# YuriPaglierani/Movie-Recommender-System-with-GNNs

Hardware: AMD Instinct MI355X
Metric: edges propagated/sec (K=3, d=64) (higher is better)
Workload: dtype fp32

## Files before the change

### include/lgcn.h

```cpp
#ifndef LGCN_H
#define LGCN_H

#include <stddef.h>
#include <stdint.h>

#ifdef __cplusplus
extern "C" {
#endif

typedef void* lgcn_stream_t;

#define LGCN_ABI_VERSION 11

#define LGCN_OK 0
#define LGCN_E_ARG (-1)
#define LGCN_E_WORKSPACE (-2)
#define LGCN_E_UNSUPPORTED (-3)

typedef struct {
    int64_t beg;
    int32_t len;
    int32_t dst;
} lgcn_item_t;

// ... 63 lines not shown
              float* partial, int32_t mode, float div, float mul,
              lgcn_stream_t stream);

int lgcn_spmm_items(const lgcn_item_t* items, int64_t n_items,
                    const lgcn_split_t* splits, int64_t n_splits,
                    const int32_t* col, const float* val, int64_t N, int32_t d,
                    const float* x_lo, const float* x_hi, int64_t x_split,
                    const float* e_lo, const float* e_hi, int64_t e_split,
                    float* y,
                    float* acc_lo, float* acc_hi, int64_t acc_split,
                    float* partial, int32_t mode, float div, float mul,
                    lgcn_stream_t stream);
int lgcn_spmm_combine(const lgcn_item_t* items, int64_t n_items,
                      const lgcn_split_t* splits, int64_t n_splits,
                      const int32_t* col, const float* val, int64_t N, int32_t d,
                      const float* x_lo, const float* x_hi, int64_t x_split,
                      const float* e_lo, const float* e_hi, int64_t e_split,
                      float* y,
                      float* acc_lo, float* acc_hi, int64_t acc_split,
                      float* partial, int32_t mode, float div, float mul,
                      lgcn_stream_t stream);
int lgcn_coalesce_workspace_size(int64_t P, int64_t N, size_t* bytes);
int lgcn_coalesce_undirected(const int64_t* src, const int64_t* dst, int64_t P, int64_t N, int64_t* out_row,
                             int64_t* out_col, int64_t* out_count, int64_t* err_count, void* ws, size_t ws_bytes,
                             lgcn_stream_t stream);

int lgcn_slice_schedule_workspace_size(int64_t E, int64_t N, int32_t S, int32_t chunk, size_t* bytes,
                                       int64_t* items_cap);
int lgcn_slice_schedule_build(const int64_t* rowptr, const int32_t* col, int64_t N, int64_t E,
                              const int64_t* bounds, int32_t S, int32_t chunk, const uint8_t* row_mask,
                              lgcn_item_t* items, int64_t items_cap,
                              int64_t* offsets, lgcn_split_t* splits, int64_t splits_cap, int64_t* counts,
                              void* ws, size_t ws_bytes, lgcn_stream_t stream);

int lgcn_spmm_run(const lgcn_item_t* items, int64_t n_items, const lgcn_split_t* splits, int64_t n_splits,
                  const int32_t* col, const float* val, int64_t N, int32_t d, const float* x_lo, const float* x_hi,
                  int64_t x_split, const float* e_lo, const float* e_hi, int64_t e_split, float* y, float* acc_lo,
                  float* acc_hi, int64_t acc_split, float* partial, int32_t mode, float div, float mul,
                  lgcn_stream_t stream, float* run);

int lgcn_spmm_run_slices(const lgcn_item_t* items, const int64_t* slice_offsets, int32_t S, const int32_t* col,
                         const float* val, int64_t N, int32_t d, const float* x_lo, const float* x_hi,
                         int64_t x_split, const float* e_lo, const float* e_hi, int64_t e_split, float* y,
                         float* acc_lo, float* acc_hi, int64_t acc_split, float* partial, int32_t mode, float div,
                         float mul, lgcn_stream_t stream, float* run);

int lgcn_spmm_blocksplit(const lgcn_item_t* items, int64_t n_items, const lgcn_split_t* splits, int64_t n_splits,
                         const int32_t* col, const float* val, int64_t N, int32_t d, const float* x_lo,
                         const float* x_hi, int64_t x_split, const float* e_lo, const float* e_hi, int64_t e_split,
                         float* y, float* acc_lo, float* acc_hi, int64_t acc_split, float* partial, int32_t mode,
                         float div, float mul, lgcn_stream_t stream, const lgcn_item_t* chunks);

typedef struct {
    const lgcn_item_t* items;
    int64_t n_items;
    const lgcn_split_t* splits;
    int64_t n_splits;
    const int32_t* col;
    const float* val;
    const float* x_lo;
    const float* x_hi;
    int64_t x_split;
    const float* e_lo;
    const float* e_hi;
    int64_t e_split;
    float* y;
// ... 279 lines not shown
```

### movie-recommender-system-with-gnns_amd/csrc/lgcn_plan.hip

```cpp

#include <hipcub/hipcub.hpp>

#include "lgcn_common.h"

using namespace lgcn;

namespace {

__global__ void k_prep_keys(const int64_t* __restrict__ key, const int64_t* __restrict__ other,
                            int64_t E, int64_t N, int32_t* __restrict__ key32,
                            int32_t* __restrict__ eid, unsigned long long* __restrict__ err) {
    const int64_t stride = int64_t(gridDim.x) * blockDim.x;
    unsigned long long bad_local = 0;
    for (int64_t e = int64_t(blockIdx.x) * blockDim.x + threadIdx.x; e < E; e += stride) {
        const int64_t k = key[e];
        const int64_t o = other[e];
        const bool bad = (k < 0) | (k >= N) | (o < 0) | (o >= N);
        bad_local += bad;
        key32[e] = bad ? 0 : static_cast<int32_t>(k);
        eid[e] = static_cast<int32_t>(e);
    }
    if (bad_local) atomicAdd(err, bad_local);
}

// ... 239 lines not shown
                sp.row = static_cast<int32_t>(i);
                sp.pbeg = part_off[i];
                sp.pcnt = n_part[i];
                sp.pad = 0;
                splits[split_off[i]] = sp;
            }
        }
        if (i == N - 1) {
            counts[0] = item_off[i] + n_items[i];
            counts[1] = split_off[i] + n_split[i];
            counts[2] = part_off[i] + n_part[i];
        }
    }
}

__global__ void k_slice_offsets(const uint32_t* __restrict__ skeys, int64_t n, int S, int64_t* __restrict__ offsets) {
    const int s = blockIdx.x * blockDim.x + threadIdx.x;
    if (s > S) return;
    const uint32_t key = static_cast<uint32_t>(s) << 24;
    int64_t lo = 0, hi = n;
    while (lo < hi) {
        const int64_t mid = (lo + hi) >> 1;
        if (skeys[mid] < key) lo = mid + 1;
        else hi = mid;
    }
    offsets[s] = lo;
}

int64_t slice_items_cap(int64_t E, int64_t N, int S, int32_t chunk) {
    const int64_t segs = E < N * int64_t(S) ? E : N * int64_t(S);
    return segs + E / chunk + N + 1;
}

__global__ void k_pair_keys(const int64_t* __restrict__ src, const int64_t* __restrict__ dst, int64_t P, int64_t N,
                            unsigned long long* __restrict__ keys, int32_t* __restrict__ bad) {
    const int64_t stride = int64_t(gridDim.x) * blockDim.x;
    for (int64_t i = int64_t(blockIdx.x) * blockDim.x + threadIdx.x; i < P; i += stride) {
        const int64_t a = src[i], b = dst[i];
        if (a < 0 || a >= N || b < 0 || b >= N) atomicOr(bad, 1);
        const int64_t ca = a < 0 ? 0 : (a >= N ? N - 1 : a);
        const int64_t cb = b < 0 ? 0 : (b >= N ? N - 1 : b);
        keys[i] = static_cast<unsigned long long>(ca) * static_cast<unsigned long long>(N) + static_cast<unsigned long long>(cb);
        keys[P + i] = static_cast<unsigned long long>(cb) * static_cast<unsigned long long>(N) + static_cast<unsigned long long>(ca);
    }
}

__global__ void k_unique_flags(const unsigned long long* __restrict__ k, int64_t n, int32_t* __restrict__ flag) {
    const int64_t stride = int64_t(gridDim.x) * blockDim.x;
    for (int64_t i = int64_t(blockIdx.x) * blockDim.x + threadIdx.x; i < n; i += stride)
        flag[i] = (i == 0 || k[i] != k[i - 1]) ? 1 : 0;
}

__global__ void k_unique_scatter(const unsigned long long* __restrict__ k, const int32_t* __restrict__ flag,
                                 const int32_t* __restrict__ pos, int64_t n, int64_t N, int64_t* __restrict__ row,
                                 int64_t* __restrict__ col, int64_t* __restrict__ count) {
    const int64_t stride = int64_t(gridDim.x) * blockDim.x;
    for (int64_t i = int64_t(blockIdx.x) * blockDim.x + threadIdx.x; i < n; i += stride) {
        if (flag[i]) {
            const unsigned long long v = k[i];
            row[pos[i]] = static_cast<int64_t>(v / static_cast<unsigned long long>(N));
            col[pos[i]] = static_cast<int64_t>(v % static_cast<unsigned long long>(N));
        }
        if (i == n - 1) count[0] = pos[i] + flag[i];
    }
}

// ... 368 lines not shown
    int32_t* i_in = c.take<int32_t>(cap);
    int32_t* i_out = c.take<int32_t>(cap);
    size_t cub_bytes = sched_cub_bytes(E, N, chunk);
    void* cub_tmp = c.take<char>(cub_bytes);
    if (!c.ok) return fail(LGCN_E_WORKSPACE, "lgcn_schedule_build: workspace %zu < %zu", ws_bytes, c.used);

    const unsigned g = grid_for(N, kBlock, 8192);
    k_sched_count<<<g, kBlock, 0, s>>>(rowptr, N, chunk, row_mask, n_items, n_part, n_split);
    if (int rc = check_launch("k_sched_count")) return rc;
    size_t t = cub_bytes;
    if (int rc = check_hip(hipcub::DeviceScan::ExclusiveSum(cub_tmp, t, n_items, item_off, static_cast<int>(N), s), "scan items")) return rc;
    t = cub_bytes;
    if (int rc = check_hip(hipcub::DeviceScan::ExclusiveSum(cub_tmp, t, n_part, part_off, static_cast<int>(N), s), "scan parts")) return rc;
    t = cub_bytes;
    if (int rc = check_hip(hipcub::DeviceScan::ExclusiveSum(cub_tmp, t, n_split, split_off, static_cast<int>(N), s), "scan splits")) return rc;
    const uint32_t pad_key = 0xFFFFFFFFu;
    k_fill_u32<<<grid_for(cap, kBlock, 8192), kBlock, 0, s>>>(k_in, cap, pad_key);
    if (int rc = check_launch("k_fill_u32")) return rc;
    k_fill_u32<<<grid_for(cap, kBlock, 8192), kBlock, 0, s>>>(reinterpret_cast<uint32_t*>(i_in), cap, 0u);
    if (int rc = check_launch("k_fill_u32")) return rc;
    k_sched_fill<<<g, kBlock, 0, s>>>(rowptr, N, chunk, side_split, n_items, item_off, n_part, part_off, n_split,
                                      split_off, raw, k_in, i_in, splits, counts);
    if (int rc = check_launch("k_sched_fill")) return rc;
    t = cub_bytes;
    if (int rc = check_hip(hipcub::DeviceRadixSort::SortPairs(cub_tmp, t, k_in, k_out, i_in, i_out,
                                                              static_cast<int>(cap), 0, 32, s),
                           "SortPairs(schedule)"))
        return rc;
    k_sched_gather<<<grid_for(cap, kBlock, 8192), kBlock, 0, s>>>(raw, i_out, cap, items);
    return check_launch("k_sched_gather");
}


int lgcn_slice_schedule_workspace_size(int64_t E, int64_t N, int32_t S, int32_t chunk, size_t* bytes,
                                       int64_t* items_cap) {
    if (!bytes || E < 0 || N < 0 || S < 1 || S > 250 || chunk < 1)
        return fail(LGCN_E_ARG, "lgcn_slice_schedule_workspace_size: bad args");
    const int64_t cap = slice_items_cap(E, N, S, chunk);
    if (items_cap) *items_cap = cap;
    size_t a = 0, b = 0, c = 0;
    (void)hipcub::DeviceScan::ExclusiveSum(nullptr, a, (const int64_t*)nullptr, (int64_t*)nullptr,
                                           static_cast<int>(N > 0 ? N : 1));
    (void)hipcub::DeviceScan::ExclusiveSum(nullptr, b, (const int32_t*)nullptr, (int32_t*)nullptr,
                                           static_cast<int>(N > 0 ? N : 1));
    (void)hipcub::DeviceRadixSort::SortPairs(nullptr, c, (const uint32_t*)nullptr, (uint32_t*)nullptr,
                                             (const int32_t*)nullptr, (int32_t*)nullptr, static_cast<int>(cap), 0,
                                             32);
    size_t m = a > b ? a : b;
    m = m > c ? m : c;
    Carver cv{nullptr, 0};
    cv.take<int64_t>(N);
    cv.take<int64_t>(N);
    cv.take<int32_t>(N);
    cv.take<int32_t>(N);
    cv.take<int32_t>(N);
    cv.take<int32_t>(N);
    cv.take<lgcn_item_t>(cap);
    cv.take<uint32_t>(cap);
    cv.take<uint32_t>(cap);
    cv.take<int32_t>(cap);
    cv.take<int32_t>(cap);
    cv.take<char>(m);
    *bytes = cv.used + 256;
    return LGCN_OK;
}

int lgcn_slice_schedule_build(const int64_t* rowptr, const int32_t* col, int64_t N, int64_t E,
                              const int64_t* bounds, int32_t S, int32_t chunk, const uint8_t* row_mask,
                              lgcn_item_t* items, int64_t items_cap,
                              int64_t* offsets, lgcn_split_t* splits, int64_t splits_cap, int64_t* counts,
                              void* ws, size_t ws_bytes, lgcn_stream_t stream) {
    if (!rowptr || !bounds || !counts || !offsets || N <= 0 || E < 0 || S < 1 || S > 250 || chunk < 1 ||
        chunk >= (1 << 24) || (E > 0 && !col))
        return fail(LGCN_E_ARG, "lgcn_slice_schedule_build: bad args");
    if (N > INT32_MAX || E > INT32_MAX) return fail(LGCN_E_UNSUPPORTED, "slice schedule: sizes exceed int32");
    hipStream_t s = as_stream(stream);
    const int64_t cap = slice_items_cap(E, N, S, chunk);
    if (!items || items_cap < cap || !splits || splits_cap < N)
        return fail(LGCN_E_ARG, "lgcn_slice_schedule_build: items_cap %lld < %lld or splits_cap %lld < %lld",
                    (long long)items_cap, (long long)cap, (long long)splits_cap, (long long)N);
    Carver c{static_cast<char*>(ws), ws_bytes};
    int64_t* n_items = c.take<int64_t>(N);
    int64_t* item_off = c.take<int64_t>(N);
    int32_t* n_part = c.take<int32_t>(N);
    int32_t* part_off = c.take<int32_t>(N);
    int32_t* n_split = c.take<int32_t>(N);
    int32_t* split_off = c.take<int32_t>(N);
    lgcn_item_t* raw = c.take<lgcn_item_t>(cap);
    uint32_t* k_in = c.take<uint32_t>(cap);
    uint32_t* k_out = c.take<uint32_t>(cap);
    int32_t* i_in = c.take<int32_t>(cap);
    int32_t* i_out = c.take<int32_t>(cap);
    size_t a = 0, b = 0, cb = 0;
    (void)hipcub::DeviceScan::ExclusiveSum(nullptr, a, (const int64_t*)nullptr, (int64_t*)nullptr, static_cast<int>(N));
    (void)hipcub::DeviceScan::ExclusiveSum(nullptr, b, (const int32_t*)nullptr, (int32_t*)nullptr, static_cast<int>(N));
    (void)hipcub::DeviceRadixSort::SortPairs(nullptr, cb, (const uint32_t*)nullptr, (uint32_t*)nullptr,
                                             (const int32_t*)nullptr, (int32_t*)nullptr, static_cast<int>(cap), 0, 32);
    size_t cub_bytes = a > b ? a : b;
    cub_bytes = cub_bytes > cb ? cub_bytes : cb;
    void* cub_tmp = c.take<char>(cub_bytes);
    if (!c.ok) return fail(LGCN_E_WORKSPACE, "lgcn_slice_schedule_build: workspace %zu < %zu", ws_bytes, c.used);
    if (int rc = check_hip(hipMemsetAsync(counts, 0, 4 * sizeof(int64_t), s), "memset counts")) return rc;
    const unsigned g = grid_for(N, kBlock, 8192);
    k_slice_count<<<grid_for(N * 64, kBlock, 8192), kBlock, 0, s>>>(rowptr, col, N, bounds, S, chunk, row_mask,
                                                                     n_items, n_part,
                                                                     n_split,
                                       reinterpret_cast<int32_t*>(counts + 3));
    if (int rc = check_launch("k_slice_count")) return rc;
    size_t t = cub_bytes;
    if (int rc = check_hip(hipcub::DeviceScan::ExclusiveSum(cub_tmp, t, n_items, item_off, static_cast<int>(N), s), "scan items")) return rc;
    t = cub_bytes;
    if (int rc = check_hip(hipcub::DeviceScan::ExclusiveSum(cub_tmp, t, n_part, part_off, static_cast<int>(N), s), "scan parts")) return rc;
    t = cub_bytes;
    if (int rc = check_hip(hipcub::DeviceScan::ExclusiveSum(cub_tmp, t, n_split, split_off, static_cast<int>(N), s), "scan splits")) return rc;
    k_fill_u32<<<grid_for(cap, kBlock, 8192), kBlock, 0, s>>>(k_in, cap, 0xFFFFFFFFu);
    if (int rc = check_launch("k_fill_u32")) return rc;
    k_fill_u32<<<grid_for(cap, kBlock, 8192), kBlock, 0, s>>>(reinterpret_cast<uint32_t*>(i_in), cap, 0u);
    if (int rc = check_launch("k_fill_u32")) return rc;
    k_slice_fill<<<g, kBlock, 0, s>>>(rowptr, col, N, bounds, S, chunk, row_mask, n_items, item_off, n_part, part_off, n_split,
                                      split_off, raw, k_in, i_in, splits, counts);
    if (int rc = check_launch("k_slice_fill")) return rc;
    t = cub_bytes;
    if (int rc = check_hip(hipcub::DeviceRadixSort::SortPairs(cub_tmp, t, k_in, k_out, i_in, i_out,
                                                              static_cast<int>(cap), 0, 32, s),
                           "SortPairs(slice schedule)"))
        return rc;
    k_sched_gather<<<grid_for(cap, kBlock, 8192), kBlock, 0, s>>>(raw, i_out, cap, items);
    if (int rc = check_launch("k_sched_gather")) return rc;
    k_slice_offsets<<<1, 256, 0, s>>>(k_out, cap, S, offsets);
    return check_launch("k_slice_offsets");
}


int lgcn_coalesce_workspace_size(int64_t P, int64_t N, size_t* bytes) {
    if (!bytes || P < 0 || N < 0) return fail(LGCN_E_ARG, "lgcn_coalesce_workspace_size: bad args");
    if (2 * P > INT32_MAX || N > (int64_t(1) << 31)) return fail(LGCN_E_UNSUPPORTED, "coalesce: sizes exceed int32");
    const int64_t n = 2 * P > 0 ? 2 * P : 1;
    Carver c{nullptr, 0};
    c.take<unsigned long long>(n);
    c.take<unsigned long long>(n);
    c.take<int32_t>(n);
    c.take<int32_t>(n);
    c.take<int32_t>(1);
    c.take<char>(coalesce_cub_bytes(n, coalesce_bits(N > 1 ? N : 2)));
    *bytes = c.used + 256;
    return LGCN_OK;
}

int lgcn_coalesce_undirected(const int64_t* src, const int64_t* dst, int64_t P, int64_t N, int64_t* out_row,
                             int64_t* out_col, int64_t* out_count, int64_t* err_count, void* ws, size_t ws_bytes,
                             lgcn_stream_t stream) {
    if (P < 0 || N <= 0 || !out_count || !err_count || (P > 0 && (!src || !dst || !out_row || !out_col)))
        return fail(LGCN_E_ARG, "lgcn_coalesce_undirected: bad args");
    if (2 * P > INT32_MAX) return fail(LGCN_E_UNSUPPORTED, "coalesce: sizes exceed int32");
    hipStream_t s = as_stream(stream);
    if (int rc = check_hip(hipMemsetAsync(out_count, 0, sizeof(int64_t), s), "memset count")) return rc;
    if (int rc = check_hip(hipMemsetAsync(err_count, 0, sizeof(int64_t), s), "memset err")) return rc;
    if (P == 0) return LGCN_OK;
    const int64_t n = 2 * P;
    const int bits = coalesce_bits(N > 1 ? N : 2);
    Carver c{static_cast<char*>(ws), ws_bytes};
    auto* k_in = c.take<unsigned long long>(n);
    auto* k_out = c.take<unsigned long long>(n);
// ... 25 lines not shown
```

### movie-recommender-system-with-gnns_amd/lgcn_amd/_ffi.py

```python
from __future__ import annotations

import ctypes
import os
import pathlib

_HERE = pathlib.Path(__file__).resolve().parent
LIB_PATH = _HERE / "liblgcn.so"

EPI_INIT = 0
EPI_ADD = 1
EPI_FINAL_ACC = 2
EPI_FINAL_E = 3
EPI_STORE = 4
EPI_SCALE = 5

E_ARG, E_WORKSPACE, E_UNSUPPORTED = -1, -2, -3

ITEM_BYTES = 16
SPLIT_BYTES = 16
ABI_VERSION = 11
DIGEST_BLOCKS = 1024
RANKED_MAX_K = 1024
RANKED_MAX_CAP = 262144
RANKED_REPEATS = -1
# ... 112 lines not shown
    "lgcn_rows_accumulate": ([_vp, _vp, _i64, _i64, _i64, _vp, _vp, _vp, _i64, _i32, _f32, _vp], ctypes.c_int),
    "lgcn_recall_width": ([_i32, _vp, _vp], ctypes.c_int),
    "lgcn_normalize_rows": ([_vp, _vp, _i64, _i64, _i32, _vp, _i32, _i64, _vp], ctypes.c_int),
    "lgcn_score_filter": ([_vp, _i64, _i64, _vp, _i64, _i64, _i32, _vp, _vp, _vp, _vp, _i32, _vp], ctypes.c_int),
    "lgcn_select_topk": ([_vp, _vp, _vp, _i32, _i32, _i32, _i64, _i64, _i64, _vp, _vp, _vp], ctypes.c_int),
    "lgcn_digest128": ([_vp, _i64, _vp, _i64, _vp, _vp], ctypes.c_int),
    "lgcn_select_topk_stl": ([_vp, _vp, _i64, _i64, _i32, _i64, _i64, _i64, _vp, _vp], ctypes.c_int),
    "lgcn_select_topk_ranked": ([_vp, _vp, _vp, _i32, _i32, _i32, _i64, _i64, _vp, _vp, _vp, _i64, _vp, _vp, _vp, _vp,
                                 _vp], ctypes.c_int),
    "lgcn_score_filter_attr": ([_vp, _i64, _i64, _vp, _i64, _i64, _i32, _vp, _vp, _vp, _vp, _i32, _vp, _vp, _vp],
                               ctypes.c_int),
    "lgcn_select_topk_ranked_attr": ([_vp, _vp, _vp, _i32, _i32, _i32, _i64, _i64, _vp, _vp, _vp, _i64, _vp, _vp, _vp,
                                      _vp, _vp, _vp, _vp], ctypes.c_int),
    "lgcn_rank_metrics": ([_vp, _i64, _i32, _i64, _vp, _vp, _vp, _i64, _vp, _i32, _vp, _vp, _vp, _vp, _vp], ctypes.c_int),
    "lgcn_rerank_mmr": ([_vp, _vp, _i64, _i32, _i64, _vp, _i64, _i32, _i32, _f32, _vp, _vp, _vp, _vp, _vp], ctypes.c_int),
    "lgcn_explain_topr": ([_vp, _i64, _i32, _i64, _vp, _vp, _vp, _vp, _i64, _vp, _i64, _i32, _i32, _vp, _vp, _vp, _vp,
                           _vp], ctypes.c_int),
    "lgcn_foldin_rows": ([_vp, _vp, _vp, _vp, _i64, _i64, _vp, _i64, _i32, _i64, _vp, _vp, _i64, _vp, _vp], ctypes.c_int),
    "lgcn_attr_profile": ([_vp, _vp, _vp, _vp, _i64, _i64, _vp, _i64, _vp, _vp, _vp], ctypes.c_int),
    "lgcn_rerank_calibrated": ([_vp, _vp, _i64, _i32, _i64, _vp, _i64, _vp, _i32, _f32, _f32, _vp, _vp, _vp, _vp, _vp],
                               ctypes.c_int),
    "lgcn_sample_negatives": ([_vp, _i64, _i64, _vp, _vp, _i64, _i64, ctypes.c_uint64, _i64, _i32, _vp, _i64, _i64, _vp,
                               _i64, _i32, _vp, _vp, _vp, _vp], ctypes.c_int),
    "lgcn_rank_positions_workspace_size": ([_i64, _i64, ctypes.POINTER(_sz)], ctypes.c_int),
    "lgcn_rank_positions": ([_vp, _i64, _i64, _vp, _i64, _i32, _vp, _vp, _vp, _i64, _vp, _vp, _vp, _i64, _vp, _i64,
                             _vp, _vp, _vp, _vp, _sz, _i32, _vp], ctypes.c_int),
    "lgcn_score_lists": ([_vp, _i64, _vp, _i64, _i32, _vp, _vp, _vp, _i64, _vp, _vp, _vp, _i32, _vp], ctypes.c_int),
    "lgcn_score_filter_groups": ([_vp, _i64, _i64, _i32, _vp, _i32, _vp, _vp, _i64, _i64, _i32, _vp, _vp, _vp, _vp, _i32,
                                  _vp], ctypes.c_int),
    "lgcn_legacy_choice": ([_vp, _vp, _i64, _i64, _i64, _vp], ctypes.c_int),
    "lgcn_slice_schedule_workspace_size": ([_i64, _i64, _i32, _i32, _vp, _vp], ctypes.c_int),
    "lgcn_slice_schedule_build": ([_vp, _vp, _i64, _i64, _vp, _i32, _i32, _vp, _vp, _i64, _vp, _vp, _i64, _vp, _vp,
                                   _sz, _vp], ctypes.c_int),
    "lgcn_coalesce_workspace_size": ([_i64, _i64, _vp], ctypes.c_int),
    "lgcn_coalesce_undirected": ([_vp, _vp, _i64, _i64, _vp, _vp, _vp, _vp, _vp, _sz, _vp], ctypes.c_int),
    "lgcn_flagged_rows_add": ([_vp, _i64, _i64, _vp, _vp, _i32, _vp, _vp, _i64, _vp], ctypes.c_int),
    "lgcn_grad_norm_workspace_floats": ([], ctypes.c_int),
    "lgcn_grad_norm": ([_vp, _i32, _f32, _vp, _vp, _vp], ctypes.c_int),
    "lgcn_adam_step": ([_vp, _i32, _f32, _f32, _f32, _f32, _f32, _f32, _vp, _vp, _i32, _vp], ctypes.c_int),
    "lgcn_adam_prologue": ([_vp, _f32, ctypes.c_double, ctypes.c_double, _vp, _vp], ctypes.c_int),
    "lgcn_program_from_graph": ([_vp, ctypes.POINTER(_vp)], ctypes.c_int),
    "lgcn_program_launches": ([_vp], ctypes.c_int),
    "lgcn_program_run": ([_vp, _vp], ctypes.c_int),
    "lgcn_program_free": ([_vp], ctypes.c_int),
    "lgcn_partition_edges": ([_vp, _vp, _i64, _i64, _i32, _i32, _f32, _vp], ctypes.c_int),
    "lgcn_partition_last_error": ([], ctypes.c_char_p),
}

EXPORTED = tuple(_SIGS)


class AdamTensor(ctypes.Structure):
    _fields_ = [("param", ctypes.c_void_p), ("grad", ctypes.c_void_p), ("exp_avg", ctypes.c_void_p),
                ("exp_avg_sq", ctypes.c_void_p), ("numel", ctypes.c_int64)]


class Pass(ctypes.Structure):
    _fields_ = [("items", ctypes.c_void_p), ("n_items", ctypes.c_int64), ("splits", ctypes.c_void_p),
                ("n_splits", ctypes.c_int64), ("col", ctypes.c_void_p), ("val", ctypes.c_void_p),
                ("x_lo", ctypes.c_void_p), ("x_hi", ctypes.c_void_p), ("x_split", ctypes.c_int64),
                ("e_lo", ctypes.c_void_p), ("e_hi", ctypes.c_void_p), ("e_split", ctypes.c_int64),
                ("y", ctypes.c_void_p), ("acc_lo", ctypes.c_void_p), ("acc_hi", ctypes.c_void_p),
                ("acc_split", ctypes.c_int64), ("partial", ctypes.c_void_p), ("mode", ctypes.c_int32),
                ("div", ctypes.c_float), ("mul", ctypes.c_float), ("n_split_big", ctypes.c_int64)]

    def __init__(self, *args, n_split_big: int = -1, **kw):
# ... 93 lines not shown
```

### movie-recommender-system-with-gnns_amd/lgcn_amd/plan.py

```python
from __future__ import annotations

import dataclasses

import torch

from . import _ffi

DEFAULT_CHUNK = 256
SLICED_CHUNK = 192
RANK_CHUNK = 128


def sliced_chunk(chunk: int) -> int:
    return min(int(chunk), SLICED_CHUNK)
BLOCK_SPLIT_MAX_CHUNKS = 32


def _block_split_for(splits: torch.Tensor, n_splits: int) -> bool:
    return n_splits == 0 or int(splits[:n_splits, 2].max().item()) <= BLOCK_SPLIT_MAX_CHUNKS


def slice_bytes_for(num_nodes: int, d: int) -> int:
    from . import tuning

# ... 165 lines not shown
        self._dst = edge_index[1].contiguous()
        stream = _ffi.stream_of(self.device)
        self.touched = None
        if touched_only:
            t = torch.zeros(self.num_nodes, dtype=torch.uint8, device=self.device)
            if self.num_edges:
                if int(edge_index.min()) < 0 or int(edge_index.max()) >= self.num_nodes:
                    raise IndexError(f"edge_index holds node ids outside [0, {self.num_nodes})")
                t[self._src] = 1
                t[self._dst] = 1
            self.touched = t
        self.fwd, self.dis, bad = _build_direction(self._dst, self._src, self.num_nodes, self.chunk,
                                                 self.side_split, None, stream, self.touched)
        if bad:
            raise IndexError(f"edge_index holds {bad} edge(s) with a node id outside [0, {self.num_nodes})")
        self._bwd: CsrDirection | None = None
        self._sched: dict = {}

    def schedule(self, which: str, d: int):
        key = (which, int(d))
        if key in self._sched:
            return self._sched[key]
        direction = self.fwd if which == "fwd" else self.bwd
        out = direction
        sb = 0 if self.touched is not None else slice_bytes_for(self.num_nodes, d)
        if sb and self.num_edges:
            from .sliced import build_sliced, slice_bounds

            bounds = slice_bounds(self.num_nodes, self.side_split, d, sb)
            from . import tuning

            forced = tuning.get().slice_mb is not None
            if forced or self.num_edges >= 8 * (len(bounds) - 1) * self.num_nodes:
                out = build_sliced(direction, self.num_nodes, bounds, sliced_chunk(direction.chunk)) or direction
        self._sched[key] = out
        return out

    @property
    def bwd(self) -> CsrDirection:
        if self._bwd is None:
            stream = _ffi.stream_of(self.device)
            self._bwd, _, _ = _build_direction(self._src, self._dst, self.num_nodes, self.chunk,
                                              self.side_split, self.dis, stream, self.touched)
        return self._bwd

    def nbytes(self) -> int:
        tot = 0
        for d in (self.fwd, self._bwd):
            if d is None:
                continue
            for t in (d.rowptr, d.col, d.eid, d.val, d.items, d.splits):
                tot += t.numel() * t.element_size()
        return tot + self.dis.numel() * 4


class PlanCache:

    def __init__(self, max_entries: int = 1024, chunk: int = DEFAULT_CHUNK):
        from ._cache import ContentLRU

        self.max_entries = max_entries
        self.chunk = chunk
        self._entries = ContentLRU(max_entries)

    def get(self, edge_index: torch.Tensor, num_nodes: int, side_split: int = 0) -> PropagationPlan:
        return self._entries.get(edge_index, lambda: PropagationPlan(edge_index, num_nodes, self.chunk, side_split),
                                 extra=(int(num_nodes), int(side_split)))
# ... 7 lines not shown
```

### movie-recommender-system-with-gnns_amd/lgcn_amd/sliced.py

```python
from __future__ import annotations

import dataclasses

import torch

from . import _ffi
from .plan import CsrDirection

MAX_SLICES = 250
ITEM_FIRST = 0x20000000
ITEM_LAST = 0x40000000


@dataclasses.dataclass
class SlicedDirection:
    base: CsrDirection
    launches: list
    splits: torch.Tensor
    n_splits: int
    n_partials: int
    bounds: list
    items: torch.Tensor = None
    host_offsets: object = None

    @property
    def n_launches(self) -> int:
        return sum(1 for _, n in self.launches if n)

    @property
    def col(self):
        return self.base.col

    @property
    def val(self):
        return self.base.val


def slice_bounds(N: int, U: int, d: int, slice_bytes: int) -> list[int]:
    out = [0]
    U = min(max(int(U), 0), N)
    for lo, hi in ((0, U), (U, N)):
        n = hi - lo
        if n <= 0:
            continue
        k = min(MAX_SLICES // 2, max(1, -(-n * d * 4 // slice_bytes)))
        if lo == U and U > 0 and n * d * 4 <= 2 * slice_bytes:
            k = 1
        out += [lo + (n * i) // k for i in range(1, k)] + [hi]
    return sorted(set(out))


def build_sliced(f: CsrDirection, N: int, bounds: list[int], chunk: int = 256,
                 row_mask: torch.Tensor | None = None) -> SlicedDirection | None:
    import ctypes

    lib = _ffi.load()
    dev = f.rowptr.device
    E = f.col.numel()
    S = len(bounds) - 1
    stream = _ffi.stream_of(dev)
    nbytes, cap = _ffi._sz(0), ctypes.c_int64(0)
    _ffi.check(lib.lgcn_slice_schedule_workspace_size(E, N, S, chunk, ctypes.byref(nbytes), ctypes.byref(cap)),
               "lgcn_slice_schedule_workspace_size")
    ws = torch.empty(max(1, nbytes.value), dtype=torch.uint8, device=dev)
    items = torch.empty((cap.value, 2), dtype=torch.int64, device=dev)
    splits = torch.empty((max(N, 1), 4), dtype=torch.int32, device=dev)
    offsets = torch.empty(S + 1, dtype=torch.int64, device=dev)
    counts = torch.zeros(4, dtype=torch.int64, device=dev)
    bnd = torch.tensor(bounds, dtype=torch.int64, device=dev)
    _ffi.check(lib.lgcn_slice_schedule_build(f.rowptr.data_ptr(), _ffi.ptr(f.col), N, E, bnd.data_ptr(), S, chunk,
                                             _ffi.ptr(row_mask), items.data_ptr(), cap.value, offsets.data_ptr(), splits.data_ptr(),
                                             splits.shape[0], counts.data_ptr(), ws.data_ptr(), ws.numel(), stream),
               "lgcn_slice_schedule_build")
    host = torch.cat([counts, offsets]).cpu().tolist()
    n_items, n_splits, n_partials, unsorted = host[:4]
    off = host[4:]
    del ws
    if unsorted:
        return None
    launches = [(items[off[s]:off[s + 1]], off[s + 1] - off[s]) for s in range(S)]
    return SlicedDirection(f, launches, splits, n_splits, n_partials, list(bounds), items,
                           (ctypes.c_int64 * (S + 1))(*off))


def _tail(sd: SlicedDirection, N, d, x, e, acc, y, mode, div, mul, partial, stream):
    xl, xh, xs = x
    el, eh, es = e if e is not None else (None, None, N)
    al, ah, as_ = acc
    return (_ffi.ptr(sd.base.col), _ffi.ptr(sd.base.val), N, d, _ffi.ptr(xl), _ffi.ptr(xh), xs, _ffi.ptr(el),
            _ffi.ptr(eh), es, _ffi.ptr(y), _ffi.ptr(al), _ffi.ptr(ah), as_, _ffi.ptr(partial), mode, div, mul, stream)


def spmm_sliced(sd: SlicedDirection, N: int, d: int, x, e, acc, y, mode: int, div: float, mul: float,
                run: torch.Tensor, partial: torch.Tensor | None, stream: int, combine: bool = True,
                timer=None) -> None:
    lib = _ffi.load()
    if sd.n_launches:
        tail = _tail(sd, N, d, x, e, acc, y, mode, div, mul, partial, stream)
        args = (sd.items.data_ptr(), sd.host_offsets, len(sd.launches), *tail, run.data_ptr())
        if timer is not None:
            with timer(d):
                rc = lib.lgcn_spmm_run_slices(*args)
        else:
            rc = lib.lgcn_spmm_run_slices(*args)
        _ffi.check(rc, "lgcn_spmm_run_slices")
    if combine:
# ... 74 lines not shown
```

### movie-recommender-system-with-gnns_amd/lgcn_amd/tuning.py

```python
from __future__ import annotations

import contextlib
import dataclasses

NATIVE = ("spmm_tail", "spmm_index_rounds", "pair_xcds_a", "partition_refine_rounds",
          "partition_cluster_rounds", "choice_threads")


@dataclasses.dataclass(frozen=True)
class Tuning:
    slice_mb: float | None = None
    slice_ride: bool = True
    neg_grouping: str = "count"
    sorted_scatter_min_b: int = 49152
    batch_chunk: int | None = None
    recall_subset: int = 16384
    recall_ties: str = "index"
    harness_fused: bool = True
    reg_in_update: bool = True
    step_program: bool = True
    device_collectives: bool = False
    spmm_tail: int = -1
    spmm_index_rounds: int = 0
    pair_xcds_a: int = 4
    partition_refine_rounds: int = 16
    partition_cluster_rounds: int = 8
    choice_threads: int = 16

    def validate(self) -> None:
        if self.slice_mb is not None and not self.slice_mb >= 0:
            raise ValueError(f"slice_mb must be None or >= 0, got {self.slice_mb}")
        if self.neg_grouping not in ("count", "radix"):
            raise ValueError(f"neg_grouping must be 'count' or 'radix', got {self.neg_grouping!r}")
        if self.sorted_scatter_min_b < 1 or self.recall_subset < 1:
            raise ValueError("sorted_scatter_min_b and recall_subset must be >= 1")
        if self.recall_ties not in ("index", "cpu"):
            raise ValueError(f"recall_ties must be 'index' or 'cpu', got {self.recall_ties!r}")
        if self.batch_chunk is not None and self.batch_chunk < 1:
            raise ValueError(f"batch_chunk must be None or >= 1, got {self.batch_chunk}")


_current = Tuning()


def get() -> Tuning:
# ... 45 lines not shown
```

Baseline: 61.61 billion.

## Deal hub-row chunks across XCDs grouped by source column within each slice

Measured after the change: 64.58 billion (median of 6 runs). 4.8% higher.

```diff
diff --git a/include/lgcn.h b/include/lgcn.h
--- a/include/lgcn.h
+++ b/include/lgcn.h
@@ -119,6 +119,13 @@
                               lgcn_item_t* items, int64_t items_cap,
                               int64_t* offsets, lgcn_split_t* splits, int64_t splits_cap, int64_t* counts,
                               void* ws, size_t ws_bytes, lgcn_stream_t stream);
+int lgcn_slice_schedule_xcd_workspace_size(int64_t E, int64_t N, int32_t S, int32_t chunk, int32_t group,
+                                           size_t* bytes, int64_t* items_cap);
+int lgcn_slice_schedule_build_xcd(const int64_t* rowptr, const int32_t* col, int64_t N, int64_t E,
+                                  const int64_t* bounds, int32_t S, int32_t chunk, int32_t group,
+                                  lgcn_item_t* items, int64_t items_cap, int64_t* offsets, lgcn_split_t* splits,
+                                  int64_t splits_cap, int64_t* counts, void* ws, size_t ws_bytes,
+                                  lgcn_stream_t stream);
 
 int lgcn_spmm_run(const lgcn_item_t* items, int64_t n_items, const lgcn_split_t* splits, int64_t n_splits,
                   const int32_t* col, const float* val, int64_t N, int32_t d, const float* x_lo, const float* x_hi,
diff --git a/movie-recommender-system-with-gnns_amd/csrc/lgcn_plan.hip b/movie-recommender-system-with-gnns_amd/csrc/lgcn_plan.hip
--- a/movie-recommender-system-with-gnns_amd/csrc/lgcn_plan.hip
+++ b/movie-recommender-system-with-gnns_amd/csrc/lgcn_plan.hip
@@ -295,6 +295,118 @@
     return segs + E / chunk + N + 1;
 }
 
+constexpr int kXcds = 8;
+constexpr uint64_t kHubPadKey = (uint64_t(0xFF) << 32) | 0xFFFFFFFFull;
+constexpr int kHubKeyBits = 40;
+
+__host__ __device__ inline int64_t hub_deal_slot(int64_t k, int64_t n, int64_t G) {
+    const int64_t rounds = (n / kXcds) / G;
+    if (rounds == 0) return k;
+    int x = static_cast<int>((k * kXcds) / n);
+    if (x > kXcds - 1) x = kXcds - 1;
+    while (x > 0 && (x * n) / kXcds > k) --x;
+    while (x < kXcds - 1 && ((x + 1) * n) / kXcds <= k) ++x;
+    const int64_t lo = (x * n) / kXcds;
+    const int64_t r = k - lo;
+    const int64_t dealt = rounds * G;
+    if (r < dealt) return ((r / G) * kXcds + x) * G + r % G;
+    return kXcds * dealt + (lo - x * dealt) + (r - dealt);
+}
+
+__global__ void k_hub_flag(const lgcn_item_t* __restrict__ items, int64_t cap, const int64_t* __restrict__ offsets,
+                           int S, int32_t chunk, int32_t* __restrict__ flag) {
+    const int64_t n_real = offsets[S];
+    const int64_t stride = int64_t(gridDim.x) * blockDim.x;
+    for (int64_t m = int64_t(blockIdx.x) * blockDim.x + threadIdx.x; m <= cap; m += stride) {
+        int32_t f = 0;
+        if (m < cap && m < n_real) {
+            const lgcn_item_t it = items[m];
+            f = (it.dst < 0 && it.len == chunk) ? 1 : 0;
+        }
+        flag[m] = f;
+    }
+}
+
+__global__ void k_fill_u64(uint64_t* __restrict__ p, int64_t n, uint64_t v) {
+    const int64_t stride = int64_t(gridDim.x) * blockDim.x;
+    for (int64_t i = int64_t(blockIdx.x) * blockDim.x + threadIdx.x; i < n; i += stride) p[i] = v;
+}
+
+__global__ void k_hub_keys(const lgcn_item_t* __restrict__ items, const uint32_t* __restrict__ skeys,
+                           const int32_t* __restrict__ flag, const int32_t* __restrict__ rank, int64_t cap,
+                           const int32_t* __restrict__ col, int64_t E, int64_t fcap, int32_t* __restrict__ pos,
+                           uint64_t* __restrict__ keys, int32_t* __restrict__ vals) {
+    const int64_t stride = int64_t(gridDim.x) * blockDim.x;
+    for (int64_t m = int64_t(blockIdx.x) * blockDim.x + threadIdx.x; m < cap; m += stride) {
+        if (!flag[m]) continue;
+        const int64_t q = rank[m];
+        const lgcn_item_t it = items[m];
+        const int64_t mid = it.beg + it.len / 2;
+        if (q < 0 || q >= fcap || mid < 0 || mid >= E) continue;
+        pos[q] = static_cast<int32_t>(m);
+        keys[q] = (uint64_t(skeys[m] >> 24) << 32) | static_cast<uint32_t>(col[mid]);
+        vals[q] = static_cast<int32_t>(m);
+    }
+}
+
+__global__ void k_hub_stage(const lgcn_item_t* __restrict__ items, const uint64_t* __restrict__ skeys64,
+                            const int32_t* __restrict__ svals, int64_t fcap, int S, int64_t cap,
+                            lgcn_item_t* __restrict__ tmp) {
+    const int64_t stride = int64_t(gridDim.x) * blockDim.x;
+    for (int64_t q = int64_t(blockIdx.x) * blockDim.x + threadIdx.x; q < fcap; q += stride) {
+        if (static_cast<int>(skeys64[q] >> 32) >= S) continue;
+        const int64_t m = svals[q];
+        if (m >= 0 && m < cap) tmp[q] = items[m];
+    }
+}
+
+__global__ void k_hub_deal(const lgcn_item_t* __restrict__ tmp, const uint64_t* __restrict__ skeys64,
+                           const int32_t* __restrict__ rank, const int64_t* __restrict__ offsets,
+                           const int32_t* __restrict__ pos, int64_t fcap, int S, int64_t cap, int32_t G,
+                           lgcn_item_t* __restrict__ items) {
+    const int64_t stride = int64_t(gridDim.x) * blockDim.x;
+    for (int64_t q = int64_t(blockIdx.x) * blockDim.x + threadIdx.x; q < fcap; q += stride) {
+        const int sl = static_cast<int>(skeys64[q] >> 32);
+        if (sl >= S) continue;
+        const int64_t o0 = offsets[sl], o1 = offsets[sl + 1];
+        if (o0 < 0 || o1 < o0 || o1 > cap) continue;
+        const int64_t base = rank[o0];
+        const int64_t n = rank[o1] - base;
+        const int64_t k = q - base;
+        if (k < 0 || k >= n) continue;
+        const int64_t slot = hub_deal_slot(k, n, G);
+        if (slot < 0 || slot >= n || base + slot >= fcap) continue;
+        const int64_t m = pos[base + slot];
+        if (m >= 0 && m < cap) items[m] = tmp[q];
+    }
+}
+
+int64_t hub_chunks_cap(int64_t E, int32_t chunk) { return E / chunk + 1; }
+
+size_t slice_cub_bytes(int64_t N, int64_t cap, int64_t fcap, int32_t G) {
+    size_t a = 0, b = 0, c = 0;
+    (void)hipcub::DeviceScan::ExclusiveSum(nullptr, a, (const int64_t*)nullptr, (int64_t*)nullptr,
+                                           static_cast<int>(N > 0 ? N : 1));
+    (void)hipcub::DeviceScan::ExclusiveSum(nullptr, b, (const int32_t*)nullptr, (int32_t*)nullptr,
+                                           static_cast<int>(N > 0 ? N : 1));
+    (void)hipcub::DeviceRadixSort::SortPairs(nullptr, c, (const uint32_t*)nullptr, (uint32_t*)nullptr,
+                                             (const int32_t*)nullptr, (int32_t*)nullptr, static_cast<int>(cap), 0,
+                                             32);
+    size_t m = a > b ? a : b;
+    m = m > c ? m : c;
+    if (G > 0) {
+        size_t e = 0, f = 0;
+        (void)hipcub::DeviceScan::ExclusiveSum(nullptr, e, (const int32_t*)nullptr, (int32_t*)nullptr,
+                                               static_cast<int>(cap + 1));
+        (void)hipcub::DeviceRadixSort::SortPairs(nullptr, f, (const uint64_t*)nullptr, (uint64_t*)nullptr,
+                                                 (const int32_t*)nullptr, (int32_t*)nullptr,
+                                                 static_cast<int>(fcap), 0, kHubKeyBits);
+        m = m > e ? m : e;
+        m = m > f ? m : f;
+    }
+    return m;
+}
+
 __global__ void k_pair_keys(const int64_t* __restrict__ src, const int64_t* __restrict__ dst, int64_t P, int64_t N,
                             unsigned long long* __restrict__ keys, int32_t* __restrict__ bad) {
     const int64_t stride = int64_t(gridDim.x) * blockDim.x;
@@ -729,22 +841,13 @@
 }
 
 
-int lgcn_slice_schedule_workspace_size(int64_t E, int64_t N, int32_t S, int32_t chunk, size_t* bytes,
-                                       int64_t* items_cap) {
-    if (!bytes || E < 0 || N < 0 || S < 1 || S > 250 || chunk < 1)
-        return fail(LGCN_E_ARG, "lgcn_slice_schedule_workspace_size: bad args");
+static int slice_ws_impl(const char* fn, int64_t E, int64_t N, int32_t S, int32_t chunk, int32_t G, size_t* bytes,
+                         int64_t* items_cap) {
+    if (!bytes || E < 0 || N < 0 || S < 1 || S > 250 || chunk < 1 || G < 0 || G > kBlock)
+        return fail(LGCN_E_ARG, "%s: bad args", fn);
     const int64_t cap = slice_items_cap(E, N, S, chunk);
+    const int64_t fcap = hub_chunks_cap(E, chunk);
     if (items_cap) *items_cap = cap;
-    size_t a = 0, b = 0, c = 0;
-    (void)hipcub::DeviceScan::ExclusiveSum(nullptr, a, (const int64_t*)nullptr, (int64_t*)nullptr,
-                                           static_cast<int>(N > 0 ? N : 1));
-    (void)hipcub::DeviceScan::ExclusiveSum(nullptr, b, (const int32_t*)nullptr, (int32_t*)nullptr,
-                                           static_cast<int>(N > 0 ? N : 1));
-    (void)hipcub::DeviceRadixSort::SortPairs(nullptr, c, (const uint32_t*)nullptr, (uint32_t*)nullptr,
-                                             (const int32_t*)nullptr, (int32_t*)nullptr, static_cast<int>(cap), 0,
-                                             32);
-    size_t m = a > b ? a : b;
-    m = m > c ? m : c;
     Carver cv{nullptr, 0};
     cv.take<int64_t>(N);
     cv.take<int64_t>(N);
@@ -757,24 +860,33 @@
     cv.take<uint32_t>(cap);
     cv.take<int32_t>(cap);
     cv.take<int32_t>(cap);
-    cv.take<char>(m);
+    cv.take<char>(slice_cub_bytes(N, cap, fcap, G));
+    if (G > 0) {
+        cv.take<int32_t>(cap + 1);
+        cv.take<int32_t>(cap + 1);
+        cv.take<int32_t>(fcap);
+        cv.take<uint64_t>(fcap);
+        cv.take<uint64_t>(fcap);
+        cv.take<int32_t>(fcap);
+        cv.take<int32_t>(fcap);
+    }
     *bytes = cv.used + 256;
     return LGCN_OK;
 }
 
-int lgcn_slice_schedule_build(const int64_t* rowptr, const int32_t* col, int64_t N, int64_t E,
-                              const int64_t* bounds, int32_t S, int32_t chunk, const uint8_t* row_mask,
-                              lgcn_item_t* items, int64_t items_cap,
-                              int64_t* offsets, lgcn_split_t* splits, int64_t splits_cap, int64_t* counts,
-                              void* ws, size_t ws_bytes, lgcn_stream_t stream) {
+static int slice_build_impl(const char* fn, const int64_t* rowptr, const int32_t* col, int64_t N, int64_t E,
+                            const int64_t* bounds, int32_t S, int32_t chunk, int32_t G, const uint8_t* row_mask,
+                            lgcn_item_t* items, int64_t items_cap, int64_t* offsets, lgcn_split_t* splits,
+                            int64_t splits_cap, int64_t* counts, void* ws, size_t ws_bytes, lgcn_stream_t stream) {
     if (!rowptr || !bounds || !counts || !offsets || N <= 0 || E < 0 || S < 1 || S > 250 || chunk < 1 ||
-        chunk >= (1 << 24) || (E > 0 && !col))
-        return fail(LGCN_E_ARG, "lgcn_slice_schedule_build: bad args");
+        chunk >= (1 << 24) || (E > 0 && !col) || G < 0 || G > kBlock)
+        return fail(LGCN_E_ARG, "%s: bad args", fn);
     if (N > INT32_MAX || E > INT32_MAX) return fail(LGCN_E_UNSUPPORTED, "slice schedule: sizes exceed int32");
     hipStream_t s = as_stream(stream);
     const int64_t cap = slice_items_cap(E, N, S, chunk);
+    const int64_t fcap = hub_chunks_cap(E, chunk);
     if (!items || items_cap < cap || !splits || splits_cap < N)
-        return fail(LGCN_E_ARG, "lgcn_slice_schedule_build: items_cap %lld < %lld or splits_cap %lld < %lld",
+        return fail(LGCN_E_ARG, "%s: items_cap %lld < %lld or splits_cap %lld < %lld", fn,
                     (long long)items_cap, (long long)cap, (long long)splits_cap, (long long)N);
     Carver c{static_cast<char*>(ws), ws_bytes};
     int64_t* n_items = c.take<int64_t>(N);
@@ -788,15 +900,20 @@
     uint32_t* k_out = c.take<uint32_t>(cap);
     int32_t* i_in = c.take<int32_t>(cap);
     int32_t* i_out = c.take<int32_t>(cap);
-    size_t a = 0, b = 0, cb = 0;
-    (void)hipcub::DeviceScan::ExclusiveSum(nullptr, a, (const int64_t*)nullptr, (int64_t*)nullptr, static_cast<int>(N));
-    (void)hipcub::DeviceScan::ExclusiveSum(nullptr, b, (const int32_t*)nullptr, (int32_t*)nullptr, static_cast<int>(N));
-    (void)hipcub::DeviceRadixSort::SortPairs(nullptr, cb, (const uint32_t*)nullptr, (uint32_t*)nullptr,
-                                             (const int32_t*)nullptr, (int32_t*)nullptr, static_cast<int>(cap), 0, 32);
-    size_t cub_bytes = a > b ? a : b;
-    cub_bytes = cub_bytes > cb ? cub_bytes : cb;
+    size_t cub_bytes = slice_cub_bytes(N, cap, fcap, G);
     void* cub_tmp = c.take<char>(cub_bytes);
-    if (!c.ok) return fail(LGCN_E_WORKSPACE, "lgcn_slice_schedule_build: workspace %zu < %zu", ws_bytes, c.used);
+    int32_t *h_flag = nullptr, *h_rank = nullptr, *h_pos = nullptr, *h_vin = nullptr, *h_vout = nullptr;
+    uint64_t *h_kin = nullptr, *h_kout = nullptr;
+    if (G > 0) {
+        h_flag = c.take<int32_t>(cap + 1);
+        h_rank = c.take<int32_t>(cap + 1);
+        h_pos = c.take<int32_t>(fcap);
+        h_kin = c.take<uint64_t>(fcap);
+        h_kout = c.take<uint64_t>(fcap);
+        h_vin = c.take<int32_t>(fcap);
+        h_vout = c.take<int32_t>(fcap);
+    }
+    if (!c.ok) return fail(LGCN_E_WORKSPACE, "%s: workspace %zu < %zu", fn, ws_bytes, c.used);
     if (int rc = check_hip(hipMemsetAsync(counts, 0, 4 * sizeof(int64_t), s), "memset counts")) return rc;
     const unsigned g = grid_for(N, kBlock, 8192);
     k_slice_count<<<grid_for(N * 64, kBlock, 8192), kBlock, 0, s>>>(rowptr, col, N, bounds, S, chunk, row_mask,
@@ -825,7 +942,62 @@
     k_sched_gather<<<grid_for(cap, kBlock, 8192), kBlock, 0, s>>>(raw, i_out, cap, items);
     if (int rc = check_launch("k_sched_gather")) return rc;
     k_slice_offsets<<<1, 256, 0, s>>>(k_out, cap, S, offsets);
-    return check_launch("k_slice_offsets");
+    if (int rc = check_launch("k_slice_offsets")) return rc;
+    if (G == 0 || E == 0) return LGCN_OK;
+
+    k_hub_flag<<<grid_for(cap + 1, kBlock, 8192), kBlock, 0, s>>>(items, cap, offsets, S, chunk, h_flag);
+    if (int rc = check_launch("k_hub_flag")) return rc;
+    t = cub_bytes;
+    if (int rc = check_hip(hipcub::DeviceScan::ExclusiveSum(cub_tmp, t, h_flag, h_rank, static_cast<int>(cap + 1), s), "scan hub chunks")) return rc;
+    k_fill_u64<<<grid_for(fcap, kBlock, 8192), kBlock, 0, s>>>(h_kin, fcap, kHubPadKey);
+    if (int rc = check_launch("k_fill_u64")) return rc;
+    k_fill_u32<<<grid_for(fcap, kBlock, 8192), kBlock, 0, s>>>(reinterpret_cast<uint32_t*>(h_vin), fcap, 0u);
+    if (int rc = check_launch("k_fill_u32")) return rc;
+    k_fill_u32<<<grid_for(fcap, kBlock, 8192), kBlock, 0, s>>>(reinterpret_cast<uint32_t*>(h_pos), fcap, 0u);
+    if (int rc = check_launch("k_fill_u32")) return rc;
+    k_hub_keys<<<grid_for(cap, kBlock, 8192), kBlock, 0, s>>>(items, k_out, h_flag, h_rank, cap, col, E, fcap, h_pos,
+                                                             h_kin, h_vin);
+    if (int rc = check_launch("k_hub_keys")) return rc;
+    t = cub_bytes;
+    if (int rc = check_hip(hipcub::DeviceRadixSort::SortPairs(cub_tmp, t, h_kin, h_kout, h_vin, h_vout,
+                                                              static_cast<int>(fcap), 0, kHubKeyBits, s),
+                           "SortPairs(hub chunks)"))
+        return rc;
+    k_hub_stage<<<grid_for(fcap, kBlock, 8192), kBlock, 0, s>>>(items, h_kout, h_vout, fcap, S, cap, raw);
+    if (int rc = check_launch("k_hub_stage")) return rc;
+    k_hub_deal<<<grid_for(fcap, kBlock, 8192), kBlock, 0, s>>>(raw, h_kout, h_rank, offsets, h_pos, fcap, S, cap, G,
+                                                              items);
+    return check_launch("k_hub_deal");
+}
+
+int lgcn_slice_schedule_workspace_size(int64_t E, int64_t N, int32_t S, int32_t chunk, size_t* bytes,
+                                       int64_t* items_cap) {
+    return slice_ws_impl("lgcn_slice_schedule_workspace_size", E, N, S, chunk, 0, bytes, items_cap);
+}
+
+int lgcn_slice_schedule_build(const int64_t* rowptr, const int32_t* col, int64_t N, int64_t E,
+                              const int64_t* bounds, int32_t S, int32_t chunk, const uint8_t* row_mask,
+                              lgcn_item_t* items, int64_t items_cap,
+                              int64_t* offsets, lgcn_split_t* splits, int64_t splits_cap, int64_t* counts,
+                              void* ws, size_t ws_bytes, lgcn_stream_t stream) {
+    return slice_build_impl("lgcn_slice_schedule_build", rowptr, col, N, E, bounds, S, chunk, 0, row_mask, items,
+                            items_cap, offsets, splits, splits_cap, counts, ws, ws_bytes, stream);
+}
+
+int lgcn_slice_schedule_xcd_workspace_size(int64_t E, int64_t N, int32_t S, int32_t chunk, int32_t group,
+                                           size_t* bytes, int64_t* items_cap) {
+    if (group < 1) return fail(LGCN_E_ARG, "lgcn_slice_schedule_xcd_workspace_size: group %d < 1", group);
+    return slice_ws_impl("lgcn_slice_schedule_xcd_workspace_size", E, N, S, chunk, group, bytes, items_cap);
+}
+
+int lgcn_slice_schedule_build_xcd(const int64_t* rowptr, const int32_t* col, int64_t N, int64_t E,
+                                  const int64_t* bounds, int32_t S, int32_t chunk, int32_t group,
+                                  lgcn_item_t* items, int64_t items_cap, int64_t* offsets, lgcn_split_t* splits,
+                                  int64_t splits_cap, int64_t* counts, void* ws, size_t ws_bytes,
+                                  lgcn_stream_t stream) {
+    if (group < 1) return fail(LGCN_E_ARG, "lgcn_slice_schedule_build_xcd: group %d < 1", group);
+    return slice_build_impl("lgcn_slice_schedule_build_xcd", rowptr, col, N, E, bounds, S, chunk, group, nullptr,
+                            items, items_cap, offsets, splits, splits_cap, counts, ws, ws_bytes, stream);
 }
 
 
diff --git a/movie-recommender-system-with-gnns_amd/lgcn_amd/_ffi.py b/movie-recommender-system-with-gnns_amd/lgcn_amd/_ffi.py
--- a/movie-recommender-system-with-gnns_amd/lgcn_amd/_ffi.py
+++ b/movie-recommender-system-with-gnns_amd/lgcn_amd/_ffi.py
@@ -168,6 +168,9 @@
     "lgcn_slice_schedule_workspace_size": ([_i64, _i64, _i32, _i32, _vp, _vp], ctypes.c_int),
     "lgcn_slice_schedule_build": ([_vp, _vp, _i64, _i64, _vp, _i32, _i32, _vp, _vp, _i64, _vp, _vp, _i64, _vp, _vp,
                                    _sz, _vp], ctypes.c_int),
+    "lgcn_slice_schedule_xcd_workspace_size": ([_i64, _i64, _i32, _i32, _i32, _vp, _vp], ctypes.c_int),
+    "lgcn_slice_schedule_build_xcd": ([_vp, _vp, _i64, _i64, _vp, _i32, _i32, _i32, _vp, _i64, _vp, _vp, _i64, _vp, _vp,
+                                       _sz, _vp], ctypes.c_int),
     "lgcn_coalesce_workspace_size": ([_i64, _i64, _vp], ctypes.c_int),
     "lgcn_coalesce_undirected": ([_vp, _vp, _i64, _i64, _vp, _vp, _vp, _vp, _vp, _sz, _vp], ctypes.c_int),
     "lgcn_flagged_rows_add": ([_vp, _i64, _i64, _vp, _vp, _i32, _vp, _vp, _i64, _vp], ctypes.c_int),
diff --git a/movie-recommender-system-with-gnns_amd/lgcn_amd/plan.py b/movie-recommender-system-with-gnns_amd/lgcn_amd/plan.py
--- a/movie-recommender-system-with-gnns_amd/lgcn_amd/plan.py
+++ b/movie-recommender-system-with-gnns_amd/lgcn_amd/plan.py
@@ -221,7 +221,8 @@
 
             forced = tuning.get().slice_mb is not None
             if forced or self.num_edges >= 8 * (len(bounds) - 1) * self.num_nodes:
-                out = build_sliced(direction, self.num_nodes, bounds, sliced_chunk(direction.chunk)) or direction
+                out = build_sliced(direction, self.num_nodes, bounds, sliced_chunk(direction.chunk),
+                                   d=d) or direction
         self._sched[key] = out
         return out
 
diff --git a/movie-recommender-system-with-gnns_amd/lgcn_amd/sliced.py b/movie-recommender-system-with-gnns_amd/lgcn_amd/sliced.py
--- a/movie-recommender-system-with-gnns_amd/lgcn_amd/sliced.py
+++ b/movie-recommender-system-with-gnns_amd/lgcn_amd/sliced.py
@@ -50,28 +50,49 @@
     return sorted(set(out))
 
 
+def items_per_workgroup(d: int) -> int:
+    if d in (4, 8, 16, 32, 64, 128, 256, 512, 1024):
+        return 256 // min(64, d // 4)
+    return 4
+
+
 def build_sliced(f: CsrDirection, N: int, bounds: list[int], chunk: int = 256,
-                 row_mask: torch.Tensor | None = None) -> SlicedDirection | None:
+                 row_mask: torch.Tensor | None = None, d: int | None = None) -> SlicedDirection | None:
     import ctypes
 
+    from . import tuning
+
     lib = _ffi.load()
+    group = items_per_workgroup(int(d)) if d is not None and row_mask is None and tuning.get().slice_hub_xcd else 0
     dev = f.rowptr.device
     E = f.col.numel()
     S = len(bounds) - 1
     stream = _ffi.stream_of(dev)
     nbytes, cap = _ffi._sz(0), ctypes.c_int64(0)
-    _ffi.check(lib.lgcn_slice_schedule_workspace_size(E, N, S, chunk, ctypes.byref(nbytes), ctypes.byref(cap)),
-               "lgcn_slice_schedule_workspace_size")
+    if group:
+        _ffi.check(lib.lgcn_slice_schedule_xcd_workspace_size(E, N, S, chunk, group, ctypes.byref(nbytes),
+                                                              ctypes.byref(cap)),
+                   "lgcn_slice_schedule_xcd_workspace_size")
+    else:
+        _ffi.check(lib.lgcn_slice_schedule_workspace_size(E, N, S, chunk, ctypes.byref(nbytes), ctypes.byref(cap)),
+                   "lgcn_slice_schedule_workspace_size")
     ws = torch.empty(max(1, nbytes.value), dtype=torch.uint8, device=dev)
     items = torch.empty((cap.value, 2), dtype=torch.int64, device=dev)
     splits = torch.empty((max(N, 1), 4), dtype=torch.int32, device=dev)
     offsets = torch.empty(S + 1, dtype=torch.int64, device=dev)
     counts = torch.zeros(4, dtype=torch.int64, device=dev)
     bnd = torch.tensor(bounds, dtype=torch.int64, device=dev)
-    _ffi.check(lib.lgcn_slice_schedule_build(f.rowptr.data_ptr(), _ffi.ptr(f.col), N, E, bnd.data_ptr(), S, chunk,
-                                             _ffi.ptr(row_mask), items.data_ptr(), cap.value, offsets.data_ptr(), splits.data_ptr(),
-                                             splits.shape[0], counts.data_ptr(), ws.data_ptr(), ws.numel(), stream),
-               "lgcn_slice_schedule_build")
+    if group:
+        _ffi.check(lib.lgcn_slice_schedule_build_xcd(f.rowptr.data_ptr(), _ffi.ptr(f.col), N, E, bnd.data_ptr(), S,
+                                                     chunk, group, items.data_ptr(), cap.value, offsets.data_ptr(),
+                                                     splits.data_ptr(), splits.shape[0], counts.data_ptr(),
+                                                     ws.data_ptr(), ws.numel(), stream),
+                   "lgcn_slice_schedule_build_xcd")
+    else:
+        _ffi.check(lib.lgcn_slice_schedule_build(f.rowptr.data_ptr(), _ffi.ptr(f.col), N, E, bnd.data_ptr(), S, chunk,
+                                                 _ffi.ptr(row_mask), items.data_ptr(), cap.value, offsets.data_ptr(), splits.data_ptr(),
+                                                 splits.shape[0], counts.data_ptr(), ws.data_ptr(), ws.numel(), stream),
+                   "lgcn_slice_schedule_build")
     host = torch.cat([counts, offsets]).cpu().tolist()
     n_items, n_splits, n_partials, unsorted = host[:4]
     off = host[4:]
diff --git a/movie-recommender-system-with-gnns_amd/lgcn_amd/tuning.py b/movie-recommender-system-with-gnns_amd/lgcn_amd/tuning.py
--- a/movie-recommender-system-with-gnns_amd/lgcn_amd/tuning.py
+++ b/movie-recommender-system-with-gnns_amd/lgcn_amd/tuning.py
@@ -11,6 +11,7 @@
 class Tuning:
     slice_mb: float | None = None
     slice_ride: bool = True
+    slice_hub_xcd: bool = True
     neg_grouping: str = "count"
     sorted_scatter_min_b: int = 49152
     batch_chunk: int | None = None
```
